# arturxe2/T-DEED

Measured on AMD Instinct MI355X. Metric: clips/sec (L=100, 224^2, bf16) forward, per-frame logits, higher is better.
Workload: dtype bf16; 1 GPU; rny002_b8: rny002_gsf + ed_sgp_mixer n_layers=2 ks=7, L=100, 224x224, batch 8/GPU, inference forward, random-init weights; clips_per_gpu=8, parallelism=dp1 (clip-sharded, no collective), hip_graph=True, batches_in_flight=3, sub_batches_per_batch=1, dist_backend=none, dist_ranks=1, self_launched=False

## Files before the change

### include/tdeed_hip.h

```cpp
#ifndef TDEED_HIP_H
#define TDEED_HIP_H
#include <stdint.h>
#ifdef __cplusplus
extern "C" {
#endif

enum { TDEED_F32 = 0, TDEED_BF16 = 1 };
enum { TDEED_ACT_NONE = 0, TDEED_ACT_RELU = 1, TDEED_ACT_GELU = 2 };
enum { TDEED_OK = 0, TDEED_ERR_ARG = -1, TDEED_ERR_LAUNCH = -2, TDEED_ERR_RUNTIME = -3 };

const char* tdeed_last_error(void);
int tdeed_abi_version(void);
int tdeed_device_info(int dev, char* name64, int* n_cu, int* is_gfx950);

int tdeed_stem_fwd(const void* frames , int frames_f32,
                   int N, int H, int W, int crop_top, int crop_left,
                   int crop_h, int crop_w, int flip ,
                   const unsigned char* flip_mask ,
                   const float* w ,
                   const float* scale , const float* shift , void* out,
                   int relu , int dtype, void* stream);

int tdeed_stem_mfma_parts(int crop_h, int crop_w);
int tdeed_stem_mfma_fwd(const void* frames, int frames_f32, int N, int H, int W, int crop_top, int crop_left, int crop_h,
                        int crop_w, int flip, const unsigned char* flip_mask, const void* wfrag, void* z, float* colpart,
                        void* stream);

int tdeed_s1_front_parts(int crop_h, int crop_w, int C1);
int tdeed_s1_front_fwd(const uint8_t* frames, int N, int H, int W, int crop_top, int crop_left, int crop_h,
                       int crop_w, int flip, const void* stem_wf, const float* stem_sc, const float* stem_sh,
                       int C1, const void* w1f, const float* sc1, const float* sh1, const void* wdf,
                       const float* scd, const float* shd, const void* w2f, const float* sc2,
                       const float* sh2, void* y2, void* shortcut, float* pooled, void* stream);

int tdeed_gemm_fwd(const void* A, long lda, const void* A0, long lda0, int k0,
                   const float* a_scale, int a_scale_rows, int M, int K, int N, const void* W,
                   long ldw, const float* scale, const float* shift, const void* R, long ldr,
                   int act, void* C, long ldc, int gather_stride, int gather_hi, int gather_wi,
                   int gather_ho, int gather_wo, float* colpart, void* C2, long ldc2, int n2, int c2_pre, int dtype,
                   void* stream);

int tdeed_gemm_ws_fits(int K, int N, int dtype);
int tdeed_gemm_ws_fwd(const void* A, long lda, const void* A0, long lda0, int k0,
                      const float* a_scale, int a_scale_rows, int M, int K, int N, const void* Wfrag,
                      const float* scale, const float* shift, const void* R, long ldr, int act,
                      void* C, long ldc, int gather_stride, int gather_hi, int gather_wi,
                      int gather_ho, int gather_wo, void* C2, long ldc2, int n2, int dtype, void* stream);

int tdeed_gconv3x3_parts(int Hi, int Wi, int C, int stride, int dtype);
int tdeed_gconv3x3_mfma_fits(int Hi, int Wi, int C, int stride);
int tdeed_gconv3x3_fwd(const void* x, int N, int Hi, int Wi, int C, int gw, int stride,
                       const float* w, const void* wfrag, const float* scale, const float* shift,
                       void* y, float* pooled, float* pooled_sq, const float* in_a, const float* in_b,
                       int relu , int dtype,
                       void* stream);

int tdeed_gemm_splitk_splits(int K);
int tdeed_gemm_splitk_partials(const void* A, long lda, int M, int K, int N, const void* W, long ldw, float* workspace,
                               void* stream);
int tdeed_gemm_splitk_fwd(const void* A, long lda, int M, int K, int N, const void* W, long ldw, const float* scale,
                          const float* shift, const void* R, long ldr, int act, void* C, long ldc,
                          float* workspace, void* stream);

int tdeed_se_gate_mfma_fits(int C, int R);
int tdeed_se_gate_mfma_fwd(const float* pooled, int n_parts, float inv_cnt, int N, int C, int R, const void* w1f,
                           const float* b1, const void* w2f, const float* b2, float* gate, void* stream);

int tdeed_gemm_rs_fits(int M, int K, int N);
int tdeed_gemm_rs_fwd(const void* A, long lda, const void* A0, long lda0, int k0, const float* a_scale, int a_scale_rows,
                      int M, int K, int N, const void* Wfrag, const float* scale, const float* shift, const void* R, long ldr,
                      int act, void* C, long ldc, void* C2, long ldc2, int n2, void* stream);

int tdeed_gemm_rs_grid(int M);
int tdeed_gemm_rs_stats_fwd(const void* A, long lda, const void* A0, long lda0, int k0, int M, int K, int N, const void* Wfrag,
                            void* C, long ldc, float* colpart, void* stream);

int tdeed_c1_gconv_set_debug(void* buf);
int tdeed_c1_gconv_fits(int Hi, int Wi, int Cin, int C, int stride);
int tdeed_c1_gconv_slab_tiles(int Hi, int Wi, int C, int stride);
int tdeed_c1_gconv_fwd(const void* x, const void* G, int Fp, int N, int Hi, int Wi, int Cin, int C, int gw, int stride,
// ... 278 lines not shown
```

### t-deed_amd/_lib.py

```python
import ctypes
import os
from ctypes import c_int, c_long, c_float, c_double, c_void_p, c_char_p, c_uint64, POINTER

import torch

CSRC = os.path.join(os.path.dirname(os.path.abspath(__file__)), "csrc")
LIB_PATH = os.path.join(CSRC, "libtdeed_hip.so")

F32, BF16 = 0, 1
ACT_NONE, ACT_RELU, ACT_GELU = 0, 1, 2


class HipLibraryMissing(RuntimeError):
    pass


class HipCallError(RuntimeError):
    pass


P = c_void_p
_SIGS = {
    "tdeed_abi_version": ([], c_int),
    "tdeed_device_info": ([c_int, c_char_p, POINTER(c_int), POINTER(c_int)], c_int),
    "tdeed_stem_fwd": ([P, c_int, c_int, c_int, c_int, c_int, c_int, c_int, c_int, c_int, P, P, P, P, P, c_int, c_int, P], c_int),
    "tdeed_augment_scratch_floats": ([c_int], c_long),
    "tdeed_augment_clips": ([P, c_int, c_int, c_int, c_int, c_int, c_int, c_int, c_int, c_int, P, P, P, P, P], c_int),
    "tdeed_mix_frames": ([P, P, P, c_int, c_long, P, P], c_int),
    "tdeed_avgpool_posenc_bwd": ([P, c_int, c_int, c_int, c_int, P, P, c_int, P], c_int),
    "tdeed_stem_mfma_parts": ([c_int, c_int], c_int),
    "tdeed_stem_mfma_fwd": ([P, c_int, c_int, c_int, c_int, c_int, c_int, c_int, c_int, c_int, P, P, P, P, P], c_int),
    "tdeed_stem_wgrad": ([P, c_int, c_int, c_int, c_int, c_int, c_int, c_int, c_int, c_int, P, P, P, P, c_int, P], c_int),
    "tdeed_stem_wgrad_bn_fits": ([c_int, c_int, c_int, c_int], c_int),
    "tdeed_stem_wgrad_bn": ([P, c_int, c_int, c_int, c_int, c_int, c_int, c_int, c_int, c_int, P, P, P, P, P, P, P, P, P, P], c_int),
    "tdeed_s1_front_parts": ([c_int, c_int, c_int], c_int),
    "tdeed_s1_front_fwd": ([P, c_int, c_int, c_int, c_int, c_int, c_int, c_int, c_int, P, P, P, c_int, P, P, P, P, P, P,
                            P, P, P, P, P, P, P], c_int),
    "tdeed_gemm_fwd": ([P, c_long, P, c_long, c_int, P, c_int, c_int, c_int, c_int, P, c_long, P, P, P, c_long,
                        c_int, P, c_long, c_int, c_int, c_int, c_int, c_int, P, P, c_long, c_int, c_int, c_int, P], c_int),
    "tdeed_gemm_ws_fits": ([c_int, c_int, c_int], c_int),
    "tdeed_gemm_ws_fwd": ([P, c_long, P, c_long, c_int, P, c_int, c_int, c_int, c_int, P, P, P, P, c_long,
                           c_int, P, c_long, c_int, c_int, c_int, c_int, c_int, P, c_long, c_int, c_int, P], c_int),
    "tdeed_gconv3x3_parts": ([c_int, c_int, c_int, c_int, c_int], c_int),
    "tdeed_gconv3x3_mfma_fits": ([c_int, c_int, c_int, c_int], c_int),
    "tdeed_gconv3x3_fwd": ([P, c_int, c_int, c_int, c_int, c_int, c_int, P, P, P, P, P, P, P, P, P, c_int, c_int, P], c_int),
    "tdeed_gemm_splitk_splits": ([c_int], c_int),
    "tdeed_gemm_splitk_fwd": ([P, c_long, c_int, c_int, c_int, P, c_long, P, P, P, c_long, c_int, P, c_long, P, P], c_int),
    "tdeed_se_gate_mfma_fits": ([c_int, c_int], c_int),
    "tdeed_se_gate_mfma_fwd": ([P, c_int, c_float, c_int, c_int, c_int, P, P, P, P, P, P], c_int),
    "tdeed_gemm_rs_fits": ([c_int, c_int, c_int], c_int),
    "tdeed_gemm_rs_grid": ([c_int], c_int),
    "tdeed_gemm_rs_stats_fwd": ([P, c_long, P, c_long, c_int, c_int, c_int, c_int, P, P, c_long, P, P], c_int),
    "tdeed_gemm_rs_fwd": ([P, c_long, P, c_long, c_int, P, c_int, c_int, c_int, c_int, P, P, P, P, c_long, c_int, P, c_long, P,
                           c_long, c_int, P], c_int),
    "tdeed_c1_gconv_set_debug": ([P], c_int),
    "tdeed_c1_gconv_fits": ([c_int, c_int, c_int, c_int, c_int], c_int),
    "tdeed_c1_gconv_slab_tiles": ([c_int, c_int, c_int, c_int], c_int),
    "tdeed_c1_gconv_fwd": ([P, P, c_int, c_int, c_int, c_int, c_int, c_int, c_int, c_int, P, P, P, P, P, P, P, P,
                            P], c_int),
    "tdeed_bneck_fits": ([c_int, c_int, c_int, c_int], c_int),
    "tdeed_bneck_set_debug": ([P], c_int),
    "tdeed_bneck_fwd": ([P, P, c_int, c_int, c_int, c_int, c_int, P, P, P, P, P, P, P, P, P, P, c_int, P, P, P, P, P, c_int,
                         c_int, P], c_int),
    "tdeed_bneck_gs_fwd": ([P, P, c_int, P, P, P, P, P, P, P, c_int, c_int, c_int, c_int, c_int, c_int, c_int, P, P, P, P, P, P, P,
                            P, P, P, c_int, P, P, P, P, P, c_int, c_int, P, P, c_int, P, P], c_int),
    "tdeed_bneck_qtail_fits": ([c_int, c_int, c_int, c_int], c_int),
    "tdeed_gsf_gate_sums_fwd": ([P, c_int, c_int, c_int, c_int, c_int, c_int, P, P, P, P, P, P], c_int),
    "tdeed_bn_slabs": ([c_long], c_int),
    "tdeed_bn_train_stats": ([P, c_long, c_int, P, P, c_float, c_float, P, P, P, P, P, P, P, c_int, P], c_int),
    "tdeed_bn_apply": ([P, c_long, c_int, P, P, P, c_int, P, c_int, P], c_int),
    "tdeed_bn_apply_slice": ([P, c_long, c_int, P, P, P, P, P, c_int, P, P, c_int, c_int, c_int, P], c_int),
    "tdeed_bn_apply2": ([P, c_long, c_int, P, P, P, P, P, c_int, P, c_int, P], c_int),
    "tdeed_bn_train_bwd": ([P, P, P, c_int, c_long, c_int, P, P, P, P, P, P, P, P, P, P, P, c_int, P], c_int),
    "tdeed_fold_rows": ([P, c_long, c_int, c_int, c_int, P, c_long, P], c_int),
    "tdeed_bn_finalize": ([P, P, c_long, c_int, c_long, c_int, P, P, c_float, c_float, P, P, P, P, P, P, P], c_int),
# ... 207 lines not shown
```

### t-deed_amd/csrc/gemm.hip

```cpp
#include "common.h"
#include <stdlib.h>

struct GemmP {
  const void* A; long lda;
  const void* A0; long lda0; int k0;
  const float* a_scale; int a_scale_rows;
  int M, K, N;
  const void* W; long ldw;
  const float* scale; const float* shift;
  const void* R; long ldr;
  int act;
  void* C; long ldc;
  int g_stride, g_hi, g_wi, g_ho, g_wo;
  float* colpart;
  void* C2; long ldc2; int n2;
  int c2_pre;
  const void* mask; long ldmask;
  const void* bz; long ldbz; const float* bmean;
  const void* bzd; long ldbzd; const float* bmean_d;
  float* bpart;
  int r_hi, r_wi;
};

template <typename T> struct Frag;
// ... 482 lines not shown
  TD_CHECK(!R || ldr % 8 == 0, "gemm_dgrad: bad residual stride");
  TD_CHECK(r_hi == 0 || (R && r_hi > 0 && r_wi > 0 && M % (r_hi * r_wi) == 0), "gemm_dgrad: bad stride-2 residual geometry");
  TD_CHECK(!mask || ldmask % 8 == 0, "gemm_dgrad: bad mask stride");
  TD_CHECK(!bpart || (bz && bmean && ldbz % 8 == 0 && (!bzd || (bmean_d && ldbzd % 8 == 0))), "gemm_dgrad: bad statistics operands");
  GemmP p{};
  p.A = A; p.lda = lda; p.a_scale_rows = 1;
  p.M = M; p.K = K; p.N = N; p.W = W; p.ldw = ldw;
  p.R = R; p.ldr = ldr; p.act = TDEED_ACT_NONE; p.C = C; p.ldc = ldc;
  p.g_stride = 1;
  p.C2 = C2; p.ldc2 = ldc2; p.n2 = C2 ? n2 : 0; p.c2_pre = C2 ? 1 : 0;
  p.mask = mask; p.ldmask = ldmask;
  p.bz = bz; p.ldbz = ldbz; p.bmean = bmean; p.bzd = bpart ? bzd : nullptr; p.ldbzd = ldbzd; p.bmean_d = bmean_d;
  p.bpart = bpart;
  p.r_hi = r_hi; p.r_wi = r_wi;
  hipStream_t st = (hipStream_t)stream;
  return dtype == TDEED_F32 ? launch_gemm<float>(p, st, true) : launch_gemm<bf16_t>(p, st, true);
}

struct GemmWsP {
  const void* A; long lda;
  const void* A0; long lda0; int k0;
  const float* a_scale; int a_scale_rows;
  int M, K, N;
  const void* Wf;
  const float* scale; const float* shift;
  const void* R; long ldr;
  int act;
  void* C; long ldc;
  int g_stride, g_hi, g_wi, g_ho, g_wo;
  int NT;
  int NTS;
  void* C2; long ldc2; int n2;
  float* colpart;
};

template <typename T, int KS, bool WLDS, int NW = 4>
__global__ __launch_bounds__(NW * 64, NW == 4 ? 2 : 1) void gemm_ws_kernel(const GemmWsP p) {
  constexpr int NTHR = NW * 64, CR = NW * 32;
  constexpr int EPC = Chunk<T>::N;
  typedef typename Frag<T>::type frag_t;
  extern __shared__ __attribute__((aligned(16))) unsigned char smem[];
  const int nt0 = WLDS ? blockIdx.y * p.NTS : 0;
  const int nts = WLDS ? min(p.NTS, p.NT - nt0) : p.NT;
  const size_t wbytes = WLDS ? (size_t)p.NTS * KS * 64 * 16 : 0;
  const frag_t* wl = WLDS ? reinterpret_cast<const frag_t*>(smem) : reinterpret_cast<const frag_t*>(p.Wf);
  float* ssc = reinterpret_cast<float*>(smem + wbytes);
  float* ssh = ssc + (WLDS ? p.NTS : p.NT) * 16;
  const int tid = threadIdx.x, lane = tid & 63, wv = tid >> 6;
  {
    if (WLDS) {
      frag_t* wdst = reinterpret_cast<frag_t*>(smem);
      const frag_t* src = reinterpret_cast<const frag_t*>(p.Wf) + (size_t)nt0 * KS * 64;
      TD_DEV_ASSERT(nts <= p.NTS && nt0 + nts <= p.NT);
      const int nfr = nts * KS * 64;
      constexpr int WB = 8;
      for (int i0 = tid; i0 < nfr; i0 += NTHR * WB) {
        frag_t v[WB];
#pragma unroll
        for (int b_ = 0; b_ < WB; ++b_) v[b_] = src[min(i0 + b_ * NTHR, nfr - 1)];
        TD_ISSUE_FENCE();
#pragma unroll
        for (int b_ = 0; b_ < WB; ++b_)
          if (i0 + b_ * NTHR < nfr) wdst[i0 + b_ * NTHR] = v[b_];
      }
    }
    for (int i = tid; i < nts * 16; i += NTHR) {
      const int n = nt0 * 16 + i;
      ssc[i] = (p.scale && n < p.N) ? p.scale[n] : 1.0f;
      ssh[i] = (p.shift && n < p.N) ? p.shift[n] : 0.0f;
    }
  }
  __syncthreads();
  const int px = lane & 15, q = lane >> 4;
  const long nchunks = ((long)p.M + CR - 1) / CR;
  for (long chunk = blockIdx.x; chunk < nchunks; chunk += gridDim.x) {
    const long mbase = chunk * CR + wv * 32;
    frag_t xf[2][KS];
    bool mok[2];
    long mrow[2];
#pragma unroll
    for (int mt = 0; mt < 2; ++mt) {
      const long m = mbase + mt * 16 + px;
      mok[mt] = m < p.M;
      const long mm = mok[mt] ? m : 0;
      mrow[mt] = mm;
      long src = mm;
      const unsigned mu = (unsigned)mm;
      if (p.g_stride > 1) {
        const unsigned per = (unsigned)(p.g_ho * p.g_wo);
        const unsigned f = mu / per, rem = mu - f * per;
        const unsigned yo = rem / (unsigned)p.g_wo, xo = rem - yo * (unsigned)p.g_wo;
        src = ((long)f * p.g_hi + (long)yo * p.g_stride) * p.g_wi + (long)xo * p.g_stride;
      }
      const T* arow = reinterpret_cast<const T*>(p.A) + src * p.lda;
      const T* a0row = p.A0 ? reinterpret_cast<const T*>(p.A0) + src * p.lda0 : nullptr;
      const float* srow = p.a_scale ? p.a_scale + (long)(mu / (unsigned)p.a_scale_rows) * (long)p.K : nullptr;
#pragma unroll
      for (int ks = 0; ks < KS; ++ks) {
        const int k = (ks * 4 + q) * EPC;
        u32x4 v = {0u, 0u, 0u, 0u};
        if (mok[mt] && k < p.K) {
          const T* s = (a0row && k < p.k0) ? a0row + k : arow + k;
          v = *reinterpret_cast<const u32x4*>(s);
          if (srow) {
            float f[EPC];
            Chunk<T>::load(reinterpret_cast<const T*>(&v), f);
#pragma unroll
            for (int e4 = 0; e4 < EPC; e4 += 4) {
              const f32x4 g4 = *reinterpret_cast<const f32x4*>(srow + k + e4);
#pragma unroll
              for (int e = 0; e < 4; ++e) f[e4 + e] *= g4[e];
            }
            Chunk<T>::store(reinterpret_cast<T*>(&v), f);
          }
        }
        xf[mt][ks] = *reinterpret_cast<frag_t*>(&v);
      }
    }
    for (int tp = 0; tp < nts; tp += 2) {
      const int chp = (nt0 + tp) * 16 + q * 8;
      u32x4 rpre[2][8 / EPC];
      if (p.R && chp < p.N) {
#pragma unroll
        for (int mt = 0; mt < 2; ++mt)
#pragma unroll
          for (int h = 0; h < 8 / EPC; ++h)
            rpre[mt][h] = *reinterpret_cast<const u32x4*>(reinterpret_cast<const T*>(p.R) + mrow[mt] * p.ldr + chp + h * EPC);
      }
      f32x4 acc[2][2];
#pragma unroll
      for (int t = 0; t < 2; ++t)
#pragma unroll
        for (int mt = 0; mt < 2; ++mt) acc[t][mt] = (f32x4){0.f, 0.f, 0.f, 0.f};
#pragma unroll
      for (int ks = 0; ks < KS; ++ks) {
        const frag_t w0 = wl[((tp + 0) * KS + ks) * 64 + lane];
        const frag_t w1 = wl[((tp + 1) * KS + ks) * 64 + lane];
#pragma unroll
        for (int mt = 0; mt < 2; ++mt) {
          acc[0][mt] = mma<T>(w0, xf[mt][ks], acc[0][mt]);
          acc[1][mt] = mma<T>(w1, xf[mt][ks], acc[1][mt]);
        }
      }
      const int ch = (nt0 + tp) * 16 + q * 8;
      if (ch < p.N) {
        float sc[8], sh[8];
#pragma unroll
        for (int e = 0; e < 8; ++e) { sc[e] = ssc[tp * 16 + q * 8 + e]; sh[e] = ssh[tp * 16 + q * 8 + e]; }
#pragma unroll
        for (int mt = 0; mt < 2; ++mt) {
          if (!mok[mt]) continue;
          float v[8];
#pragma unroll
          for (int r = 0; r < 4; ++r) {
            v[r] = acc[0][mt][r] * sc[r] + sh[r];
            v[4 + r] = acc[1][mt][r] * sc[4 + r] + sh[4 + r];
          }
          const long m = mrow[mt];
          if (p.R) {
            float rv[EPC];
#pragma unroll
            for (int h = 0; h < 8 / EPC; ++h) {
              Chunk<T>::load(reinterpret_cast<const T*>(&rpre[mt][h]), rv);
#pragma unroll
              for (int e = 0; e < EPC; ++e) v[h * EPC + e] += rv[e];
            }
          }
          if (p.act == TDEED_ACT_RELU) {
#pragma unroll
            for (int e = 0; e < 8; ++e) v[e] = fmaxf(v[e], 0.f);
          } else if (p.act == TDEED_ACT_GELU) {
#pragma unroll
            for (int e = 0; e < 8; ++e) v[e] = gelu_erf(v[e]);
          }
          T* cp = reinterpret_cast<T*>(p.C) + m * p.ldc + ch;
          T* cp2 = (p.C2 && ch < p.n2) ? reinterpret_cast<T*>(p.C2) + m * p.ldc2 + ch : nullptr;
#pragma unroll
          for (int h = 0; h < 8 / EPC; ++h) {
            float o[EPC];
#pragma unroll
            for (int e = 0; e < EPC; ++e) o[e] = v[h * EPC + e];
            Chunk<T>::store(cp + h * EPC, o);
            if (cp2) Chunk<T>::store(cp2 + h * EPC, o);
          }
        }
      }
    }
  }
}

static size_t ws_lds_cap() {
  static const size_t cap = [] {
// ... 82 lines not shown
  return 0;
}

extern "C" int tdeed_gemm_ws_fwd(const void* A, long lda, const void* A0, long lda0, int k0,
                                 const float* a_scale, int a_scale_rows, int M, int K, int N,
                                 const void* Wfrag, const float* scale, const float* shift, const void* R,
                                 long ldr, int act, void* C, long ldc, int gather_stride, int gather_hi,
                                 int gather_wi, int gather_ho, int gather_wo, void* C2, long ldc2, int n2, int dtype,
                                 void* stream) {
  TD_CHECK(A && Wfrag && C, "gemm_ws: null pointer");
  TD_CHECK(!C2 || (n2 > 0 && n2 % 8 == 0 && n2 <= N && ldc2 % 8 == 0 && ldc2 >= n2),
           "gemm_ws: bad second output n2=%d ldc2=%ld", n2, ldc2);
  TD_CHECK(M > 0 && K > 0 && N > 0, "gemm_ws: bad sizes M=%d K=%d N=%d", M, K, N);
  TD_CHECK(dtype == TDEED_F32 || dtype == TDEED_BF16, "gemm_ws: bad dtype %d", dtype);
  TD_CHECK(K % 8 == 0 && N % 8 == 0 && lda % 8 == 0 && ldc % 8 == 0, "gemm_ws: K, N, lda, ldc must be multiples of 8");
  TD_CHECK(!A0 || (k0 % 8 == 0 && lda0 % 8 == 0 && k0 <= K), "gemm_ws: bad splice");
  TD_CHECK(!R || ldr % 8 == 0, "gemm_ws: bad ldr");
  TD_CHECK(act >= 0 && act <= 2, "gemm_ws: bad act %d", act);
  TD_CHECK(tdeed_gemm_ws_fits(K, N, dtype), "gemm_ws: K=%d N=%d does not fit the weight-stationary kernel", K, N);
  if (gather_stride > 1)
    TD_CHECK(gather_hi > 0 && gather_wi > 0 && gather_ho > 0 && gather_wo > 0 && M % (gather_ho * gather_wo) == 0,
             "gemm_ws: bad gather geometry");
  GemmWsP p{};
  p.A = A; p.lda = lda; p.A0 = A0; p.lda0 = lda0; p.k0 = A0 ? k0 : 0;
  p.a_scale = a_scale; p.a_scale_rows = a_scale_rows > 0 ? a_scale_rows : 1;
  p.M = M; p.K = K; p.N = N; p.Wf = Wfrag; p.scale = scale; p.shift = shift;
  p.R = R; p.ldr = ldr; p.act = act; p.C = C; p.ldc = ldc;
  p.g_stride = gather_stride; p.g_hi = gather_hi; p.g_wi = gather_wi; p.g_ho = gather_ho; p.g_wo = gather_wo;
  p.NT = (N + 31) / 32 * 2;
  p.NTS = p.NT;
  p.C2 = C2; p.ldc2 = ldc2; p.n2 = C2 ? n2 : 0;
  hipStream_t st = (hipStream_t)stream;
  return dtype == TDEED_F32 ? launch_gemm_ws<float>(p, st) : launch_gemm_ws<bf16_t>(p, st);
}

constexpr int RS_KS = 10, RS_NW = 10, RS_THR = RS_NW * 64, RS_ROWS = 64, RS_LD = RS_KS * 64 + 96;
constexpr int RS_TILE = RS_ROWS * RS_LD;
constexpr int RS_CPT = RS_ROWS * RS_KS * 4 / RS_THR;
constexpr int RS_KSR = 8;
constexpr int RS_WTAIL = RS_NW * 2 * (RS_KS - RS_KSR) * 64 * 16;

template <bool SE, bool RES, bool OUT2, bool STATS = false>
__global__ __launch_bounds__(RS_THR, 1) void gemm_rs_kernel(const GemmWsP p) {
  typedef bf16_t T;
  extern __shared__ __attribute__((aligned(16))) unsigned char smem[];
  unsigned char* tiles = smem;
  bf16x8* wtail = reinterpret_cast<bf16x8*>(smem + 2 * RS_TILE);
  float* gt = reinterpret_cast<float*>(smem + 2 * RS_TILE + RS_WTAIL);
  float* bnt = gt + 4 * RS_KS * 32;
  const int tid = threadIdx.x, lane = tid & 63, wv = __builtin_amdgcn_readfirstlane(tid >> 6);
  const int px = lane & 15, q = lane >> 4;
  const int KP = RS_KS * 32;
  bf16x8 wf[2][RS_KSR];
  bf16x8* wt = wtail + wv * 2 * (RS_KS - RS_KSR) * 64 + lane;
#pragma unroll
  for (int h = 0; h < 2; ++h)
#pragma unroll
    for (int ks = 0; ks < RS_KS; ++ks) {
      const bf16x8 f = reinterpret_cast<const bf16x8*>(p.Wf)[((long)(2 * wv + h) * RS_KS + ks) * 64 + lane];
      if (ks < RS_KSR) wf[h][ks] = f;
      else wt[(h * (RS_KS - RS_KSR) + ks - RS_KSR) * 64] = f;
    }
  for (int i = tid; i < 2 * p.N; i += RS_THR) {
    const int n = i % p.N;
    bnt[i] = i < p.N ? (p.scale ? p.scale[n] : 1.0f) : (p.shift ? p.shift[n] : 0.0f);
  }
// ... 528 lines not shown
```

### t-deed_amd/engine.py

```python
import os
from types import SimpleNamespace

import numpy as np
import torch

from . import ops, _lib
from .streams import new_stream
from .regnet_spec import regnet_spec, sgp_up_size, pyramid_lengths
from .packing import (_np, _f32, _dense, pack_ws_weights, pack_se_bf16, pack_mfma_frags, pack_se_mfma,
                      pack_front_weights, _stem_frags_np, gs_source_order_columns, _gsf_q_frags_np, pack_gsf_q_frags,
                      _gsf_p_frags_np, pack_gsf_p_frags, pack_gconv_frags, _gconv_frags_np, stem_frags_on_device,
                      gsf_q_frags_on_device, gconv_frag_index, gconv_frags_on_device)

BN_EPS = 1e-5


class _Pool:

    def __init__(self, device):
        self.device = device
        self.free = []
        self.all = []

    def take(self, shape, dtype):
# ... 104 lines not shown
    return o


def pack_sgp_mixer(sd, pre, C, act_dtype, device):
    o = SimpleNamespace(C=C)
    for n in ("ln1", "ln2"):
        setattr(o, n + "_w", _f32(_np(sd[f"{pre}.{n}.weight"]).reshape(C), device))
        setattr(o, n + "_b", _f32(_np(sd[f"{pre}.{n}.bias"]).reshape(C), device))
    o.dw1, o.db1 = _dwpack(sd, pre, ["psi1", "convw1", "convkw1", "fc1", "global_fc1"], C, device)
    o.dw2, o.db2 = _dwpack(sd, pre, ["psi2", "convw2", "convkw2", "fc2", "global_fc2"], C, device)
    o.ks = _np(sd[pre + ".psi1.weight"]).shape[-1]
    o.up = _np(sd[pre + ".convkw1.weight"]).shape[-1]
    o.w_cat = _dense(_np(sd[pre + ".concat_fc.weight"]).reshape(C, 6 * C), act_dtype, device)
    o.b_cat = _f32(_np(sd[pre + ".concat_fc.bias"]), device)
    o.wcg = (pack_mfma_frags(_np(sd[pre + ".concat_fc.weight"]).reshape(C, 6 * C), device, ks_mult=12)
             if act_dtype == torch.bfloat16 and str(device) != "cpu" and C % 16 == 0 and SGP_GEMM else None)
    _pack_mlp(sd, pre, C, o, act_dtype, device)
    return o


def _se(pooled, inv_cnt, bw, gate):
    if bw.se_mf is not None:
        return ops.se_gate_mfma(pooled, inv_cnt, bw.se_mf.w1f, bw.se_b1, bw.se_mf.w2f, bw.se_b2, bw.spec.se_rd, out=gate)
    if bw.se_bf is not None:
        return ops.se_gate_bf16(pooled, inv_cnt, bw.se_bf.se_w1p, bw.se_b1, bw.se_bf.se_w2p, bw.se_b2, bw.spec.se_rd, out=gate)
    return ops.se_gate(pooled, inv_cnt, bw.se_w1t, bw.se_b1, bw.se_w2t, bw.se_b2, out=gate)


BNECK_ONE_LAUNCH = os.environ.get("TDEED_BNECK", "1") == "1"
BNECK_BLEND = True
BNECK_QTAIL = True
C1_GCONV = os.environ.get("TDEED_C1_GCONV", "1") == "1"
C1_GCONV_MAX_CIN = 160


def _bneck_fused(bw, h, w, out_is_slice):
    blk = bw.spec
    return bool(BNECK_ONE_LAUNCH and getattr(bw, "fused", None) is not None and bw.se_mf is not None and blk.stride == 1
                and not blk.has_downsample and blk.cin == blk.cout and not out_is_slice
                and ops.bneck_fits(h, w, blk.cout, blk.se_rd))


class Step:
    __slots__ = ("name", "kernel", "fn", "bytes", "flops")

    def __init__(self, name, kernel, fn, nbytes=0, flops=0):
        self.name, self.kernel, self.fn, self.bytes, self.flops = name, kernel, fn, int(nbytes), int(flops)


def _esz(dt):
    return 2 if dt == torch.bfloat16 else 4


def gemm_cost(M, K, N, es, residual=False, extra=0):
    return (M * K + N * K + M * N * (2 if residual else 1)) * es + extra, 2 * M * K * N


class SgpBuilder:

    def __init__(self, pool, steps, keep, taps, B, act_dtype):
        self.pool, self.steps, self.keep, self.taps, self.B, self.dt = pool, steps, keep, taps, B, act_dtype
        self.splitk_rows = 4096
        self.fused = os.environ.get("TDEED_SGP_FUSED", "1") == "1"
        self.gemm = SGP_GEMM and act_dtype == torch.bfloat16

    def _mlp_gemm(self, name, y, o, Tn, chsum, pool_to=None, y16=None):
# ... 301 lines not shown
        self.W = W


_DEAD_GRAPHS = []
_CAPTURING = 0


def _drain_dead_graphs():
    if not _DEAD_GRAPHS or _CAPTURING:
        return
    torch.cuda.synchronize()
    while _DEAD_GRAPHS:
        _lib.call("tdeed_graph_destroy", _DEAD_GRAPHS.pop())


class ForwardEngine:
    def __init__(self, cfg, state, act_dtype=torch.bfloat16, device="cuda", use_graph=True, fuse_front=True, n_split=2):
        if not torch.cuda.is_available():
            raise RuntimeError("tdeed_amd.ForwardEngine needs an MI355X (no CPU path)")
        _lib.load()
        self.cfg = cfg
        g = (lambda k: cfg[k]) if isinstance(cfg, dict) else (lambda k: getattr(cfg, k))
        self.crop_dim = g("crop_dim")
        self.pw = PackedWeights(cfg, state, act_dtype, device)
        self.act_dtype = act_dtype
        self.device = device
        self.use_graph = use_graph
        self.fuse_front = fuse_front
        self.n_split = int(os.environ.get("TDEED_SPLIT", n_split))
        self.merge_tail = True
        self.join_at = None
        self._plans = {}

    def _se_conv3(self, bw, N, h2, w2, y2, pooled, gate, sc, out, out2=None):
        blk, es, M2 = bw.spec, _esz(self.act_dtype), N * h2 * w2
        return (Step(blk.name + ".se", "se_gate", lambda: _se(pooled, 1.0 / (h2 * w2), bw, gate),
                     2 * N * blk.cout * 4 + 2 * blk.cout * blk.se_rd * 4, 4 * N * blk.cout * blk.se_rd),
                Step(blk.name + ".conv3", bw.w3.kern(M2), lambda: bw.w3.run(
                    y2, bw.s3, bw.h3, ops.ACT_RELU, residual=sc, a_scale=gate, a_scale_rows=h2 * w2, out=out, M=M2, out2=out2),
                    *gemm_cost(M2, blk.cout, blk.cout, es, True)))

    @staticmethod
    def _block_done(pool, keep, taps, blk, dead, x, x_kept, out):
        for t_ in dead:
            pool.give(t_)
        if not x_kept and hasattr(x, "_td_raw"):
            pool.give(x)
        tapname = "_features." + blk.name
        if tapname in taps:
            keep[tapname] = out
        return tapname in taps

    def _avgpool(self, steps, B, x, h, w, feat, frs=None):
        pw, Wt = self.pw, self.pw.W
        N, C = B * pw.clip_len, pw.spec.feat_dim
        if frs is None:
            frs = torch.empty((N, 2), dtype=torch.float32, device=self.device)
        feat._td_rowstat = frs
        steps.append(Step("avgpool", "avgpool_posenc", lambda: ops.avgpool_posenc(x, B, pw.clip_len, Wt.temp_enc, out=feat,
                                                                                 rowstat=frs),
                          (N * h * w + N) * C * _esz(self.act_dtype)))

    def _sgp_heads(self, pool, steps, keep, taps, B, feat, head_out):
        pw, Wt = self.pw, self.pw.W
        N, C = B * pw.clip_len, pw.spec.feat_dim
        cur = SgpBuilder(pool, steps, keep, taps, B, self.act_dtype).pyramid(feat, pw.clip_len, pw.n_layers, Wt.sgp, Wt.mixer)
        steps.append(Step("heads", "heads", lambda: ops.heads(cur, Wt.head_w, Wt.head_b, out=head_out),
                          N * C * _esz(self.act_dtype) + N * pw.n_out * 4, 2 * N * C * pw.n_out))
        return cur

    def _blocks(self, pool, steps, keep, taps, B, x, h, w, blocks, x_kept, out_last=None):
        pw, Wt = self.pw, self.pw.W
        T = pw.clip_len
# ... 64 lines not shown
                    run = lambda x=x, xg=xg, bw=bw, gb=gb, out=out, o2=o2, F=F, Fp=Fp, qt=qt: ops.bneck_gs(
                        x, xg, gb["gate"], gb["ysum"], gb["xsum"], bw.gs_cw1, bw.gs_cb1, bw.gs_cw2, bw.gs_cb2, T, F, Fp,
                        bw.fused.w1f, bw.s1, bw.h1, bw.fused.w2f, bw.s2, bw.h2, bw.se_mf.w1f, bw.se_b1, bw.se_mf.w2f, bw.se_b2,
                        bw.spec.se_rd, bw.fused.w3f, bw.s3, bw.h3, out=out, out2=o2, w2_tap_major=bw.fused.w2_tap_major, qtail=qt)
                else:
                    run = lambda x=x, bw=bw, G=G, out=out, o2=o2: ops.bneck(
                        x, bw.fused.w1f, bw.s1, bw.h1, bw.fused.w2f, bw.s2, bw.h2, bw.se_mf.w1f, bw.se_b1, bw.se_mf.w2f, bw.se_b2,
                        bw.spec.se_rd, bw.fused.w3f, bw.s3, bw.h3, G=G, out=out, out2=o2, w2_tap_major=bw.fused.w2_tap_major)
                steps.append(Step(blk.name + ".bneck", "bneck", run,
                                  (2 * M * blk.cout + (M * Fp if blend_in else 0)) * es + (8 * M if blend_in else 0)
                                  + (24 * M if (blend_in and qt is not None) else 0)
                                  + (2 * blk.cout * blk.cout + blk.cout * blk.gw * 9) * es,
                                  2 * M * blk.cout * (2 * blk.cout + blk.gw * 9)))
                x_kept = self._block_done(pool, keep, taps, blk, gs_bufs, x, x_kept, out)
                xs, x = xs_next, out
                continue
            s = blk.stride
            h2, w2 = (h - 1) // s + 1, (w - 1) // s + 1
            M2 = N * h2 * w2
            y2 = pool.take((N, h2, w2, blk.cout), dt)
            parts = ops.gconv3x3_parts(h, w, blk.cout, s, dt) if bw.w2frag is not None else 1
            pooled = pool.take((N, parts, blk.cout), torch.float32)
            gate = pool.take((N, blk.cout), torch.float32)
            if c1g:
                G = gb["out"] if blk.gsf_fold else None
                steps.append(Step(blk.name + ".conv1_conv2", "c1_gconv", lambda x=x, bw=bw, blk=blk, G=G, y2=y2, pooled=pooled: ops.c1_gconv(
                    x, bw.c1g_w1f, bw.s1, bw.h1, bw.w2frag, bw.s2, bw.h2, blk.gw, blk.stride, blk.cout, G=G, out=y2, pooled=pooled),
                    (M * blk.cin + M2 * blk.cout) * es + blk.cout * (blk.cin + blk.gw * 9) * es,
                    2 * M * blk.cin * blk.cout + 2 * M2 * blk.cout * blk.gw * 9))
            else:
                steps.append(Step(blk.name + ".conv2", "gconv3x3", lambda y1=y1, bw=bw, blk=blk, y2=y2, pooled=pooled: ops.gconv3x3(
                    y1, bw.w2, bw.s2, bw.h2, blk.gw, blk.stride, wfrag=bw.w2frag, out=y2, pooled=pooled),
                    (M + M2) * blk.cout * es + blk.cout * blk.gw * 9 * 4, 2 * M2 * blk.cout * blk.gw * 9))
            sc, shortcut = x, []
            if blk.has_downsample:
                sc = pool.take((N, h2, w2, blk.cout), dt)
                gather = (s, h, w, h2, w2) if s > 1 else None
                shortcut = [Step(blk.name + ".downsample", bw.wd.kern(M2), lambda x=x, bw=bw, sc=sc, gather=gather, M2=M2: bw.wd.run(
                    x, bw.sd, bw.hd, ops.ACT_NONE, gather=gather, out=sc, M=M2),
                    *gemm_cost(M2, blk.cin, blk.cout, es))]
            out = (out_last if (out_last is not None and bw is blocks[-1]) else pool.take((N, h2, w2, blk.cout), dt))
            nxt = blocks[bi + 1].spec if bi + 1 < len(blocks) else None
            xs_next = None
            if nxt is not None and nxt.gsf_fold and GS_SLICE:
                xs_next = pool.take((N, h2, w2, (nxt.gsf_fold + 7) // 8 * 8), dt)
            se, conv3 = self._se_conv3(bw, N, h2, w2, y2, pooled, gate, sc, out, out2=xs_next)
            steps += [se, *shortcut, conv3]
            dead = ([y1] if y1 is not None else []) + [y2, pooled, gate] + gs_bufs + ([sc] if blk.has_downsample else [])
            x_kept = self._block_done(pool, keep, taps, blk, dead, x, x_kept, out)
            xs, x, h, w = xs_next, out, h2, w2
        return x, h, w, x_kept

    def _build_tail(self, B, feat, head_out, trunk_in=None, start=None):
        pool, steps, keep = _Pool(self.device), [], {}
        if trunk_in is not None:
            x, h, w = trunk_in
            x, h, w, _ = self._blocks(pool, steps, keep, set(), B, x, h, w, list(self.pw.W.blocks[start:]), True)
            self._avgpool(steps, B, x, h, w, feat)
        cur = self._sgp_heads(pool, steps, keep, set(), B, feat, head_out)
        return SimpleNamespace(steps=steps, pool_bytes=pool.total_bytes(), sgp_out=cur)

    def _build(self, B, H, W, flip, taps, head_out=None, feat_out=None, stop_at=None, trunk_out=None, feat_rs=None,
               frames_dtype=torch.uint8):
        pw, Wt = self.pw, self.pw.W
        T = pw.clip_len
        N = B * T
        dt = self.act_dtype
        dev = self.device
        pool = _Pool(dev)
        steps = []
        keep = {}
        crop = None
        ch, cw = H, W
        if self.crop_dim is not None and self.crop_dim > 0 and (self.crop_dim != H or self.crop_dim != W):
            ch = cw = self.crop_dim
            crop = (int(round((H - ch) / 2.0)), int(round((W - cw) / 2.0)), ch, cw)
        frames = torch.empty((N, 3, H, W), dtype=frames_dtype, device=dev)
        Ho, Wo = (ch + 1) // 2, (cw + 1) // 2
        es = _esz(dt)
        blocks = list(Wt.blocks)
        fused_front = (Wt.front is not None and "_features.stem" not in taps and self.fuse_front
# ... 223 lines not shown
```

### t-deed_amd/ops.py

```python
import ctypes

import torch

from . import _lib
from ._lib import call, ptr, stream_ptr, dtype_code, ACT_NONE, ACT_RELU, ACT_GELU


def _chk(t, name, dtype=None):
    if t is None:
        return
    if not t.is_cuda:
        raise RuntimeError(f"{name} must be a GPU tensor (tdeed_amd has no CPU path)")
    if not t.is_contiguous():
        raise RuntimeError(f"{name} must be contiguous")
    if dtype is not None and t.dtype != dtype:
        raise TypeError(f"{name}: expected {dtype}, got {t.dtype}")


def _flip_args(flip, N):
    if isinstance(flip, torch.Tensor):
        m = flip.to(torch.uint8).contiguous()
        if m.numel() != N or not m.is_cuda:
            raise ValueError(f"flip mask must hold one flag per frame on the GPU ({m.numel()} vs {N})")
        return 0, m
# ... 150 lines not shown
def gsq_bn_table(bn_scale, bn_shift):
    F = bn_scale.numel()
    t = torch.zeros((2, (F + 7) // 8 * 8), dtype=torch.float32, device=bn_scale.device)
    t[0, :F] = bn_scale
    t[1, :F] = bn_shift
    return t


def gemm_ws_fits_mode(K, N, act_dtype):
    return _lib.load().tdeed_gemm_ws_fits(K, N, dtype_code(act_dtype))


def gemm_ws_fits(K, N, act_dtype):
    return gemm_ws_fits_mode(K, N, act_dtype) != 0


def gemm_ws(A, Wfrag, K, N, scale=None, shift=None, act=ACT_NONE, residual=None, a_scale=None, a_scale_rows=0,
            A0=None, k0=0, gather=None, out=None, M=None, lda=None, ldc=None, out2=None):
    _chk(A, "A")
    if M is None:
        M = A.numel() // A.shape[-1]
        if gather is not None:
            s, hi, wi, ho, wo = gather
            M = (M // (hi * wi)) * ho * wo
    lda = A.shape[-1] if lda is None else lda
    if out is None:
        out = torch.empty((M, N), dtype=A.dtype, device=A.device)
    ldc = N if ldc is None else ldc
    g = gather if gather is not None else (1, 0, 0, 0, 0)
    call("tdeed_gemm_ws_fwd", ptr(A), lda, ptr(A0), (A0.shape[-1] if A0 is not None else 0), k0,
         ptr(a_scale), a_scale_rows, M, K, N, ptr(Wfrag), ptr(scale), ptr(shift),
         ptr(residual), (residual.shape[-1] if residual is not None else 0), act, ptr(out), ldc,
         g[0], g[1], g[2], g[3], g[4], *_out2(out2, A), dtype_code(A.dtype), stream_ptr())
    return out


def gemm_rs_fits(M, K, N):
    return _lib.load().tdeed_gemm_rs_fits(M, K, N) != 0


def gemm_rs(A, Wfrag, K, N, scale=None, shift=None, act=ACT_NONE, residual=None, a_scale=None, a_scale_rows=0, A0=None, k0=0,
            out=None, M=None, out2=None):
    _chk(A, "A", torch.bfloat16)
    if M is None:
        M = A.numel() // A.shape[-1]
    if out is None:
        out = torch.empty((M, N), dtype=A.dtype, device=A.device)
    call("tdeed_gemm_rs_fwd", ptr(A), A.shape[-1], ptr(A0), (A0.shape[-1] if A0 is not None else 0), k0, ptr(a_scale),
         a_scale_rows, M, K, N, ptr(Wfrag), ptr(scale), ptr(shift), ptr(residual),
         (residual.shape[-1] if residual is not None else 0), act, ptr(out), N, *_out2(out2, A), stream_ptr())
    return out


def gemm_rs_stats(A, Wfrag, K, N, M=None, A0=None, k0=0):
    _chk(A, "A", torch.bfloat16)
    if M is None:
        M = A.numel() // A.shape[-1]
    out = torch.empty((M, N), dtype=A.dtype, device=A.device)
    P = _lib.load().tdeed_gemm_rs_grid(M)
    cp = torch.empty((P, 2, N), dtype=torch.float32, device=A.device)
    call("tdeed_gemm_rs_stats_fwd", ptr(A), A.shape[-1], ptr(A0), (A0.shape[-1] if A0 is not None else 0), k0, M, K, N,
         ptr(Wfrag), ptr(out), N, ptr(cp), stream_ptr())
    flat = cp.view(-1)
    return out, (flat, flat[N:], 2 * N, P)


# ... 480 lines not shown
```

Before: 5330 clips/s.

## Fuse downsample shortcut GEMM into conv3 GEMM as second operand

Adds a two-operand weight-stationary GEMM variant that computes the strided downsample projection of the block input alongside conv3. The projection result is rounded through bf16 and added as the residual in the epilogue. This removes a separate downsample kernel launch and the write and re-read of the shortcut tensor. In exchange it uses more LDS per block, which can lower occupancy, and it only covers two K shapes.

New measurement: 5508 clips/s, median of 6. 1.03x the previous value.

```diff
diff --git a/include/tdeed_hip.h b/include/tdeed_hip.h
--- a/include/tdeed_hip.h
+++ b/include/tdeed_hip.h
@@ -46,6 +46,14 @@
                       const float* scale, const float* shift, const void* R, long ldr, int act,
                       void* C, long ldc, int gather_stride, int gather_hi, int gather_wi,
                       int gather_ho, int gather_wo, void* C2, long ldc2, int n2, int dtype, void* stream);
+
+int tdeed_gemm_ws_sc_fits(int K, int Ks, int N, int dtype);
+int tdeed_gemm_ws_sc_fwd(const void* A, long lda, const void* A0, long lda0, int k0, const float* a_scale,
+                         int a_scale_rows, int M, int K, int N, const void* Wfrag, const float* scale,
+                         const float* shift, const void* As, long ldas, int Ks, const void* Wsfrag,
+                         const float* sscale, const float* sshift, int act, void* C, long ldc, int gather_stride,
+                         int gather_hi, int gather_wi, int gather_ho, int gather_wo, void* C2, long ldc2, int n2,
+                         int dtype, void* stream);
 
 int tdeed_gconv3x3_parts(int Hi, int Wi, int C, int stride, int dtype);
 int tdeed_gconv3x3_mfma_fits(int Hi, int Wi, int C, int stride);
diff --git a/t-deed_amd/_lib.py b/t-deed_amd/_lib.py
--- a/t-deed_amd/_lib.py
+++ b/t-deed_amd/_lib.py
@@ -41,6 +41,9 @@
     "tdeed_gemm_ws_fits": ([c_int, c_int, c_int], c_int),
     "tdeed_gemm_ws_fwd": ([P, c_long, P, c_long, c_int, P, c_int, c_int, c_int, c_int, P, P, P, P, c_long,
                            c_int, P, c_long, c_int, c_int, c_int, c_int, c_int, P, c_long, c_int, c_int, P], c_int),
+    "tdeed_gemm_ws_sc_fits": ([c_int, c_int, c_int, c_int], c_int),
+    "tdeed_gemm_ws_sc_fwd": ([P, c_long, P, c_long, c_int, P, c_int, c_int, c_int, c_int, P, P, P, P, c_long, c_int, P, P, P,
+                              c_int, P, c_long, c_int, c_int, c_int, c_int, c_int, P, c_long, c_int, c_int, P], c_int),
     "tdeed_gconv3x3_parts": ([c_int, c_int, c_int, c_int, c_int], c_int),
     "tdeed_gconv3x3_mfma_fits": ([c_int, c_int, c_int, c_int], c_int),
     "tdeed_gconv3x3_fwd": ([P, c_int, c_int, c_int, c_int, c_int, c_int, P, P, P, P, P, P, P, P, P, c_int, c_int, P], c_int),
diff --git a/t-deed_amd/csrc/gemm.hip b/t-deed_amd/csrc/gemm.hip
--- a/t-deed_amd/csrc/gemm.hip
+++ b/t-deed_amd/csrc/gemm.hip
@@ -538,9 +538,26 @@
   int NTS;
   void* C2; long ldc2; int n2;
   float* colpart;
+  const void* As; long ldas; int Ks;
+  const void* Wsf;
+  const float* sscale; const float* sshift;
 };
 
-template <typename T, int KS, bool WLDS, int NW = 4>
+template <typename frag_t, int NTHR>
+__device__ __forceinline__ void ws_fill_frags(frag_t* wdst, const frag_t* src, int nfr, int tid) {
+  constexpr int WB = 8;
+  for (int i0 = tid; i0 < nfr; i0 += NTHR * WB) {
+    frag_t v[WB];
+#pragma unroll
+    for (int b_ = 0; b_ < WB; ++b_) v[b_] = src[min(i0 + b_ * NTHR, nfr - 1)];
+    TD_ISSUE_FENCE();
+#pragma unroll
+    for (int b_ = 0; b_ < WB; ++b_)
+      if (i0 + b_ * NTHR < nfr) wdst[i0 + b_ * NTHR] = v[b_];
+  }
+}
+
+template <typename T, int KS, bool WLDS, int NW = 4, int KS2 = 0>
 __global__ __launch_bounds__(NW * 64, NW == 4 ? 2 : 1) void gemm_ws_kernel(const GemmWsP p) {
   constexpr int NTHR = NW * 64, CR = NW * 32;
   constexpr int EPC = Chunk<T>::N;
@@ -552,28 +569,28 @@
   const frag_t* wl = WLDS ? reinterpret_cast<const frag_t*>(smem) : reinterpret_cast<const frag_t*>(p.Wf);
   float* ssc = reinterpret_cast<float*>(smem + wbytes);
   float* ssh = ssc + (WLDS ? p.NTS : p.NT) * 16;
+  const frag_t* wl2 = reinterpret_cast<const frag_t*>(ssh + p.NTS * 16);
+  float* ssc2 = reinterpret_cast<float*>(smem + wbytes + (size_t)p.NTS * 128 + (size_t)p.NTS * KS2 * 64 * 16);
+  float* ssh2 = ssc2 + p.NTS * 16;
+  static_assert(KS2 == 0 || WLDS, "the two-operand form keeps both weights in LDS");
   const int tid = threadIdx.x, lane = tid & 63, wv = tid >> 6;
   {
     if (WLDS) {
       frag_t* wdst = reinterpret_cast<frag_t*>(smem);
       const frag_t* src = reinterpret_cast<const frag_t*>(p.Wf) + (size_t)nt0 * KS * 64;
       TD_DEV_ASSERT(nts <= p.NTS && nt0 + nts <= p.NT);
-      const int nfr = nts * KS * 64;
-      constexpr int WB = 8;
-      for (int i0 = tid; i0 < nfr; i0 += NTHR * WB) {
-        frag_t v[WB];
-#pragma unroll
-        for (int b_ = 0; b_ < WB; ++b_) v[b_] = src[min(i0 + b_ * NTHR, nfr - 1)];
-        TD_ISSUE_FENCE();
-#pragma unroll
-        for (int b_ = 0; b_ < WB; ++b_)
-          if (i0 + b_ * NTHR < nfr) wdst[i0 + b_ * NTHR] = v[b_];
-      }
+      ws_fill_frags<frag_t, NTHR>(wdst, src, nts * KS * 64, tid);
+      if constexpr (KS2 > 0)
+        ws_fill_frags<frag_t, NTHR>(const_cast<frag_t*>(wl2), reinterpret_cast<const frag_t*>(p.Wsf), nts * KS2 * 64, tid);
     }
     for (int i = tid; i < nts * 16; i += NTHR) {
       const int n = nt0 * 16 + i;
       ssc[i] = (p.scale && n < p.N) ? p.scale[n] : 1.0f;
       ssh[i] = (p.shift && n < p.N) ? p.shift[n] : 0.0f;
+      if constexpr (KS2 > 0) {
+        ssc2[i] = (p.sscale && n < p.N) ? p.sscale[n] : 1.0f;
+        ssh2[i] = (p.sshift && n < p.N) ? p.sshift[n] : 0.0f;
+      }
     }
   }
   __syncthreads();
@@ -582,6 +599,7 @@
   for (long chunk = blockIdx.x; chunk < nchunks; chunk += gridDim.x) {
     const long mbase = chunk * CR + wv * 32;
     frag_t xf[2][KS];
+    frag_t xs[2][KS2 > 0 ? KS2 : 1];
     bool mok[2];
     long mrow[2];
 #pragma unroll
@@ -598,6 +616,17 @@
         const unsigned yo = rem / (unsigned)p.g_wo, xo = rem - yo * (unsigned)p.g_wo;
         src = ((long)f * p.g_hi + (long)yo * p.g_stride) * p.g_wi + (long)xo * p.g_stride;
       }
+      if constexpr (KS2 > 0) {
+        const T* srow2 = reinterpret_cast<const T*>(p.As) + src * p.ldas;
+#pragma unroll
+        for (int ks = 0; ks < KS2; ++ks) {
+          const int k = (ks * 4 + q) * EPC;
+          u32x4 v = {0u, 0u, 0u, 0u};
+          if (mok[mt] && k < p.Ks) v = *reinterpret_cast<const u32x4*>(srow2 + k);
+          xs[mt][ks] = *reinterpret_cast<frag_t*>(&v);
+        }
+        src = mm;
+      }
       const T* arow = reinterpret_cast<const T*>(p.A) + src * p.lda;
       const T* a0row = p.A0 ? reinterpret_cast<const T*>(p.A0) + src * p.lda0 : nullptr;
       const float* srow = p.a_scale ? p.a_scale + (long)(mu / (unsigned)p.a_scale_rows) * (long)p.K : nullptr;
@@ -626,7 +655,7 @@
     for (int tp = 0; tp < nts; tp += 2) {
       const int chp = (nt0 + tp) * 16 + q * 8;
       u32x4 rpre[2][8 / EPC];
-      if (p.R && chp < p.N) {
+      if (KS2 == 0 && p.R && chp < p.N) {
 #pragma unroll
         for (int mt = 0; mt < 2; ++mt)
 #pragma unroll
@@ -646,6 +675,23 @@
         for (int mt = 0; mt < 2; ++mt) {
           acc[0][mt] = mma<T>(w0, xf[mt][ks], acc[0][mt]);
           acc[1][mt] = mma<T>(w1, xf[mt][ks], acc[1][mt]);
+        }
+      }
+      f32x4 accs[2][2];
+      if constexpr (KS2 > 0) {
+#pragma unroll
+        for (int t = 0; t < 2; ++t)
+#pragma unroll
+          for (int mt = 0; mt < 2; ++mt) accs[t][mt] = (f32x4){0.f, 0.f, 0.f, 0.f};
+#pragma unroll
+        for (int ks = 0; ks < KS2; ++ks) {
+          const frag_t w0 = wl2[((tp + 0) * KS2 + ks) * 64 + lane];
+          const frag_t w1 = wl2[((tp + 1) * KS2 + ks) * 64 + lane];
+#pragma unroll
+          for (int mt = 0; mt < 2; ++mt) {
+            accs[0][mt] = mma<T>(w0, xs[mt][ks], accs[0][mt]);
+            accs[1][mt] = mma<T>(w1, xs[mt][ks], accs[1][mt]);
+          }
         }
       }
       const int ch = (nt0 + tp) * 16 + q * 8;
@@ -663,7 +709,25 @@
             v[4 + r] = acc[1][mt][r] * sc[4 + r] + sh[4 + r];
           }
           const long m = mrow[mt];
-          if (p.R) {
+          if constexpr (KS2 > 0) {
+            float sv[8];
+#pragma unroll
+            for (int r = 0; r < 4; ++r) {
+              sv[r] = accs[0][mt][r] * ssc2[tp * 16 + q * 8 + r] + ssh2[tp * 16 + q * 8 + r];
+              sv[4 + r] = accs[1][mt][r] * ssc2[tp * 16 + q * 8 + 4 + r] + ssh2[tp * 16 + q * 8 + 4 + r];
+            }
+#pragma unroll
+            for (int h = 0; h < 8 / EPC; ++h) {
+              u32x4 rb;
+              float rv[EPC];
+#pragma unroll
+              for (int e = 0; e < EPC; ++e) rv[e] = sv[h * EPC + e];
+              Chunk<T>::store(reinterpret_cast<T*>(&rb), rv);
+              Chunk<T>::load(reinterpret_cast<const T*>(&rb), rv);
+#pragma unroll
+              for (int e = 0; e < EPC; ++e) v[h * EPC + e] += rv[e];
+            }
+          } else if (p.R) {
             float rv[EPC];
 #pragma unroll
             for (int h = 0; h < 8 / EPC; ++h) {
@@ -812,6 +876,75 @@
   p.C2 = C2; p.ldc2 = ldc2; p.n2 = C2 ? n2 : 0;
   hipStream_t st = (hipStream_t)stream;
   return dtype == TDEED_F32 ? launch_gemm_ws<float>(p, st) : launch_gemm_ws<bf16_t>(p, st);
+}
+
+static constexpr size_t WS_SC_LDS_MAX = 80 * 1024;
+static size_t ws_sc_smem(int NT, int KS, int KS2) {
+  return (size_t)NT * (KS + KS2) * 64 * 16 + (size_t)NT * 16 * 4 * sizeof(float);
+}
+extern "C" int tdeed_gemm_ws_sc_fits(int K, int Ks, int N, int dtype) {
+  if (dtype != TDEED_BF16 || K <= 0 || Ks <= 0 || N <= 0) return 0;
+  const int KS = (K + 31) / 32, KS2 = (Ks + 31) / 32, NT = (N + 31) / 32 * 2;
+  if (!((KS == 2 && KS2 == 1) || (KS == 5 && KS2 == 2))) return 0;
+  return ws_sc_smem(NT, KS, KS2) <= WS_SC_LDS_MAX;
+}
+
+template <int KS, int KS2>
+static int launch_gemm_ws_sc(const GemmWsP& p, hipStream_t st) {
+  const size_t smem = ws_sc_smem(p.NT, KS, KS2);
+  static TdDevOnce attr_set;
+  if (smem > 64 * 1024 && !attr_set.get()) {
+    if (hipFuncSetAttribute((const void*)gemm_ws_kernel<bf16_t, KS, true, 4, KS2>, hipFuncAttributeMaxDynamicSharedMemorySize,
+                            (int)WS_SC_LDS_MAX) != hipSuccess) {
+      tdeed_set_error("gemm_ws_sc: hipFuncSetAttribute failed");
+      return TDEED_ERR_RUNTIME;
+    }
+    attr_set.set();
+  }
+  const long nchunks = ((long)p.M + 127) / 128;
+  long per_cu = (long)((160 * 1024) / smem);
+  if (per_cu > 4) per_cu = 4;
+  long gx = 256 * per_cu;
+  if (gx > nchunks) gx = nchunks;
+  hipLaunchKernelGGL((gemm_ws_kernel<bf16_t, KS, true, 4, KS2>), dim3((unsigned)gx, 1), dim3(256), smem, st, p);
+  TD_LAUNCH_CHECK("gemm_ws_sc");
+  return TDEED_OK;
+}
+
+extern "C" int tdeed_gemm_ws_sc_fwd(const void* A, long lda, const void* A0, long lda0, int k0, const float* a_scale,
+                                    int a_scale_rows, int M, int K, int N, const void* Wfrag, const float* scale,
+                                    const float* shift, const void* As, long ldas, int Ks, const void* Wsfrag,
+                                    const float* sscale, const float* sshift, int act, void* C, long ldc, int gather_stride,
+                                    int gather_hi, int gather_wi, int gather_ho, int gather_wo, void* C2, long ldc2, int n2,
+                                    int dtype, void* stream) {
+  TD_CHECK(A && Wfrag && C && As && Wsfrag, "gemm_ws_sc: null pointer");
+  TD_CHECK(!C2 || (n2 > 0 && n2 % 8 == 0 && n2 <= N && ldc2 % 8 == 0 && ldc2 >= n2),
+           "gemm_ws_sc: bad second output n2=%d ldc2=%ld", n2, ldc2);
+  TD_CHECK(M > 0 && K > 0 && N > 0 && Ks > 0, "gemm_ws_sc: bad sizes M=%d K=%d N=%d Ks=%d", M, K, N, Ks);
+  TD_CHECK(dtype == TDEED_BF16, "gemm_ws_sc: bf16 only (dtype %d)", dtype);
+  TD_CHECK(K % 8 == 0 && N % 8 == 0 && Ks % 8 == 0 && lda % 8 == 0 && ldc % 8 == 0 && ldas % 8 == 0 && lda >= K && ldas >= Ks &&
+               ldc >= N,
+           "gemm_ws_sc: K, N, Ks, lda, ldc, ldas must be multiples of 8 and the strides cover the rows");
+  TD_CHECK(!A0 || (k0 % 8 == 0 && lda0 % 8 == 0 && k0 <= K && lda0 >= k0), "gemm_ws_sc: bad splice");
+  TD_CHECK(act >= 0 && act <= 2, "gemm_ws_sc: bad act %d", act);
+  TD_CHECK(tdeed_gemm_ws_sc_fits(K, Ks, N, dtype), "gemm_ws_sc: K=%d Ks=%d N=%d is not one of the two-operand forms", K, Ks, N);
+  if (gather_stride > 1)
+    TD_CHECK(gather_hi > 0 && gather_wi > 0 && gather_ho > 0 && gather_wo > 0 && M % (gather_ho * gather_wo) == 0 &&
+                 (long)(gather_ho - 1) * gather_stride < gather_hi && (long)(gather_wo - 1) * gather_stride < gather_wi,
+             "gemm_ws_sc: bad gather geometry");
+  GemmWsP p{};
+  p.A = A; p.lda = lda; p.A0 = A0; p.lda0 = lda0; p.k0 = A0 ? k0 : 0;
+  p.a_scale = a_scale; p.a_scale_rows = a_scale_rows > 0 ? a_scale_rows : 1;
+  p.M = M; p.K = K; p.N = N; p.Wf = Wfrag; p.scale = scale; p.shift = shift;
+  p.act = act; p.C = C; p.ldc = ldc;
+  p.g_stride = gather_stride > 1 ? gather_stride : 1;
+  p.g_hi = gather_hi; p.g_wi = gather_wi; p.g_ho = gather_ho; p.g_wo = gather_wo;
+  p.NT = (N + 31) / 32 * 2;
+  p.NTS = p.NT;
+  p.C2 = C2; p.ldc2 = ldc2; p.n2 = C2 ? n2 : 0;
+  p.As = As; p.ldas = ldas; p.Ks = Ks; p.Wsf = Wsfrag; p.sscale = sscale; p.sshift = sshift;
+  hipStream_t st = (hipStream_t)stream;
+  return (K + 31) / 32 == 2 ? launch_gemm_ws_sc<2, 1>(p, st) : launch_gemm_ws_sc<5, 2>(p, st);
 }
 
 constexpr int RS_KS = 10, RS_NW = 10, RS_THR = RS_NW * 64, RS_ROWS = 64, RS_LD = RS_KS * 64 + 96;
diff --git a/t-deed_amd/engine.py b/t-deed_amd/engine.py
--- a/t-deed_amd/engine.py
+++ b/t-deed_amd/engine.py
@@ -160,6 +160,7 @@
 BNECK_QTAIL = True
 C1_GCONV = os.environ.get("TDEED_C1_GCONV", "1") == "1"
 C1_GCONV_MAX_CIN = 160
+SC_IN_CONV3 = True
 
 
 def _bneck_fused(bw, h, w, out_is_slice):
@@ -527,13 +528,20 @@
         self.join_at = None
         self._plans = {}
 
-    def _se_conv3(self, bw, N, h2, w2, y2, pooled, gate, sc, out, out2=None):
+    def _se_conv3(self, bw, N, h2, w2, y2, pooled, gate, sc, out, out2=None, sc_from=None):
         blk, es, M2 = bw.spec, _esz(self.act_dtype), N * h2 * w2
-        return (Step(blk.name + ".se", "se_gate", lambda: _se(pooled, 1.0 / (h2 * w2), bw, gate),
-                     2 * N * blk.cout * 4 + 2 * blk.cout * blk.se_rd * 4, 4 * N * blk.cout * blk.se_rd),
-                Step(blk.name + ".conv3", bw.w3.kern(M2), lambda: bw.w3.run(
-                    y2, bw.s3, bw.h3, ops.ACT_RELU, residual=sc, a_scale=gate, a_scale_rows=h2 * w2, out=out, M=M2, out2=out2),
-                    *gemm_cost(M2, blk.cout, blk.cout, es, True)))
+        se = Step(blk.name + ".se", "se_gate", lambda: _se(pooled, 1.0 / (h2 * w2), bw, gate),
+                  2 * N * blk.cout * 4 + 2 * blk.cout * blk.se_rd * 4, 4 * N * blk.cout * blk.se_rd)
+        if sc_from is not None:
+            x, gather = sc_from
+            return (se, Step(blk.name + ".conv3", "gemm_ws", lambda: ops.gemm_ws_sc(
+                y2, bw.w3.w, blk.cout, blk.cout, bw.s3, bw.h3, x, bw.wd.w, blk.cin, bw.sd, bw.hd, ops.ACT_RELU, a_scale=gate,
+                a_scale_rows=h2 * w2, gather=gather, out=out, M=M2, out2=out2),
+                (M2 * (2 * blk.cout + blk.cin) + blk.cout * (blk.cout + blk.cin)) * es,
+                2 * M2 * blk.cout * (blk.cout + blk.cin)))
+        return (se, Step(blk.name + ".conv3", bw.w3.kern(M2), lambda: bw.w3.run(
+            y2, bw.s3, bw.h3, ops.ACT_RELU, residual=sc, a_scale=gate, a_scale_rows=h2 * w2, out=out, M=M2, out2=out2),
+            *gemm_cost(M2, blk.cout, blk.cout, es, True)))
 
     @staticmethod
     def _block_done(pool, keep, taps, blk, dead, x, x_kept, out):
@@ -664,10 +672,13 @@
                 steps.append(Step(blk.name + ".conv2", "gconv3x3", lambda y1=y1, bw=bw, blk=blk, y2=y2, pooled=pooled: ops.gconv3x3(
                     y1, bw.w2, bw.s2, bw.h2, blk.gw, blk.stride, wfrag=bw.w2frag, out=y2, pooled=pooled),
                     (M + M2) * blk.cout * es + blk.cout * blk.gw * 9 * 4, 2 * M2 * blk.cout * blk.gw * 9))
-            sc, shortcut = x, []
-            if blk.has_downsample:
+            sc, shortcut, sc_from = x, [], None
+            gather = (s, h, w, h2, w2) if s > 1 else None
+            if (SC_IN_CONV3 and blk.has_downsample and dt == torch.bfloat16 and bw.w3.ws and bw.wd.ws
+                    and ops.gemm_ws_sc_fits(blk.cout, blk.cin, blk.cout, dt)):
+                sc, sc_from = None, (x, gather)
+            elif blk.has_downsample:
                 sc = pool.take((N, h2, w2, blk.cout), dt)
-                gather = (s, h, w, h2, w2) if s > 1 else None
                 shortcut = [Step(blk.name + ".downsample", bw.wd.kern(M2), lambda x=x, bw=bw, sc=sc, gather=gather, M2=M2: bw.wd.run(
                     x, bw.sd, bw.hd, ops.ACT_NONE, gather=gather, out=sc, M=M2),
                     *gemm_cost(M2, blk.cin, blk.cout, es))]
@@ -676,9 +687,9 @@
             xs_next = None
             if nxt is not None and nxt.gsf_fold and GS_SLICE:
                 xs_next = pool.take((N, h2, w2, (nxt.gsf_fold + 7) // 8 * 8), dt)
-            se, conv3 = self._se_conv3(bw, N, h2, w2, y2, pooled, gate, sc, out, out2=xs_next)
+            se, conv3 = self._se_conv3(bw, N, h2, w2, y2, pooled, gate, sc, out, out2=xs_next, sc_from=sc_from)
             steps += [se, *shortcut, conv3]
-            dead = ([y1] if y1 is not None else []) + [y2, pooled, gate] + gs_bufs + ([sc] if blk.has_downsample else [])
+            dead = ([y1] if y1 is not None else []) + [y2, pooled, gate] + gs_bufs + ([sc] if shortcut else [])
             x_kept = self._block_done(pool, keep, taps, blk, dead, x, x_kept, out)
             xs, x, h, w = xs_next, out, h2, w2
         return x, h, w, x_kept
diff --git a/t-deed_amd/ops.py b/t-deed_amd/ops.py
--- a/t-deed_amd/ops.py
+++ b/t-deed_amd/ops.py
@@ -206,6 +206,32 @@
          ptr(a_scale), a_scale_rows, M, K, N, ptr(Wfrag), ptr(scale), ptr(shift),
          ptr(residual), (residual.shape[-1] if residual is not None else 0), act, ptr(out), ldc,
          g[0], g[1], g[2], g[3], g[4], *_out2(out2, A), dtype_code(A.dtype), stream_ptr())
+    return out
+
+
+def gemm_ws_sc_fits(K, Ks, N, act_dtype):
+    lib = _lib.load()
+    if not hasattr(lib, "tdeed_gemm_ws_sc_fits"):
+        return False
+    return lib.tdeed_gemm_ws_sc_fits(K, Ks, N, dtype_code(act_dtype)) != 0
+
+
+def gemm_ws_sc(A, Wfrag, K, N, scale, shift, As, Wsfrag, Ks, sscale, sshift, act=ACT_NONE, a_scale=None, a_scale_rows=0,
+               A0=None, k0=0, gather=None, out=None, M=None, out2=None):
+    _chk(A, "A", torch.bfloat16); _chk(As, "As", torch.bfloat16)
+    if M is None:
+        M = A.numel() // A.shape[-1]
+    rows_s = As.numel() // As.shape[-1]
+    g = gather if gather is not None else (1, 0, 0, 0, 0)
+    need = (M // (g[3] * g[4])) * g[1] * g[2] if gather is not None else M
+    if rows_s < need or A.numel() // A.shape[-1] < M:
+        raise ValueError(f"gemm_ws_sc: operands hold {A.numel() // A.shape[-1]} / {rows_s} rows, {M} / {need} needed")
+    if out is None:
+        out = torch.empty((M, N), dtype=A.dtype, device=A.device)
+    call("tdeed_gemm_ws_sc_fwd", ptr(A), A.shape[-1], ptr(A0), (A0.shape[-1] if A0 is not None else 0), k0,
+         ptr(a_scale), a_scale_rows, M, K, N, ptr(Wfrag), ptr(scale), ptr(shift), ptr(As), As.shape[-1], Ks, ptr(Wsfrag),
+         ptr(sscale), ptr(sshift), act, ptr(out), N, g[0], g[1], g[2], g[3], g[4], *_out2(out2, A), dtype_code(A.dtype),
+         stream_ptr())
     return out
 
 
```
